# FederatedAI/FATE-LLM

Measured on AMD Instinct MI355X. Metric: GB/s param buffer reconstructed from (seed,scalar) list, device-resident, higher is better.
Workload: dtype bf16

## Files before the change

### fate-llm_amd/csrc/fks_device.hip

```cpp
#include <hip/hip_runtime.h>
#include <hip/hip_bf16.h>

#include <type_traits>

#include "fks_internal.h"
#include "fks_bitslice.h"
#define FKS_HD __device__ __forceinline__
#include "fks_libm.h"

constexpr int kDbMinWaves = 4;
constexpr int kZrUnroll = 2;
constexpr int kSm2MinWaves = 8;
constexpr int kBsFence = 8;
#ifndef FKS_BS_LAG
#define FKS_BS_LAG 36
#endif
#ifndef FKS_BS_R_VMEM
#define FKS_BS_R_VMEM 3
#endif
#ifndef FKS_BS_D16
#define FKS_BS_D16 1
#endif
#ifndef FKS_BS_G32
#define FKS_BS_G32 1
#endif
#ifndef FKS_BS_ROWMIN
#define FKS_BS_ROWMIN 1
#endif
#ifndef FKS_BS_FLIPMUX
#define FKS_BS_FLIPMUX 1
#endif
#ifndef FKS_PHX_VEC_ITEMS
#define FKS_PHX_VEC_ITEMS 8
#endif
#ifndef FKS_BS_WGTIME
#define FKS_BS_WGTIME 0
#endif

#include "fks_dev_lds.h"
#include "fks_dev_update.h"
#include "fks_dev_mt.h"
#include "fks_dev_zgen.h"
#include "fks_dev_irr.h"
#include "fks_dev_host.h"
#include "fks_kern_jump.h"
#include "fks_kern_apply.h"
#include "fks_kern_slice.h"
#include "fks_kern_irregular.h"
#include "fks_kern_philox.h"
#include "fks_kern_selfcheck.h"

namespace fks {

int launch_delta_apply(const DeltaApplyDesc* d, int n, int64_t max_numel, const float* delta, void* stream) {
  const int64_t blocks = std::min<int64_t>(std::max<int64_t>(1, (max_numel + 255) / 256), 2048);
  hipLaunchKernelGGL(fks_delta_apply_kernel, dim3((unsigned)blocks, (unsigned)n), dim3(256), 0, (hipStream_t)stream,
                     d, delta);
  return (int)hipGetLastError();
}

static size_t apply_lds_bytes() { return (size_t)kLdsTabBytes + (size_t)kLdsStBytes; }

int device_cu_count() {
  int dev = 0, n = 0;
  if (hipGetDevice(&dev) != hipSuccess) return 256;
  if (hipDeviceGetAttribute(&n, hipDeviceAttributeMultiprocessorCount, dev) != hipSuccess || n <= 0) return 256;
  return n;
}

template <int... Vs>
struct IntList {};
template <int... Vs, class F>
static int dispatch(IntList<Vs...>, int v, F&& f) {
  int r = -FKS_ENOTSUP;
  (void)((v == Vs && (r = f(std::integral_constant<int, Vs>{}), true)) || ...);
  return r;
}

int launch_jump(const JumpArgs& a, int nseeds, void* stream) {
  const size_t lds = sizeof(uint32_t) * (size_t)kJumpLds2Words;
  static PerDevice attr;
  if (int e = ensure_lds_attr(attr, &fks_jump_kernel, (int)lds)) return e;
  dim3 grid((unsigned)nseeds, (unsigned)((a.nchunks + a.chunks_per_wg - 1) / a.chunks_per_wg));
// ... 27 lines not shown
static int launch_apply_t(const ApplyArgs& a, void* stream) {
  if (a.nseeds == kMaxSeedsPerPass) return launch_apply_f<DT, MODE, true>(a, stream);
  if constexpr (DT == FKS_BF16) {
    if (a.zmode == 1 && a.nseeds == 1 && MODE == kModePerturb) return launch_small2<DT, MODE, 1>(a, stream);
    if (a.zmode == 2 && a.nseeds == 1 &&
        (MODE == kModePerturb || MODE == kModePerturbUpdate || MODE == kModeUpdate || MODE == kModeUpdateWd ||
         MODE == kModeUpdateNoWd || MODE == kModeUpdateWd0)) {
      hipLaunchKernelGGL((fks_zreplay_kernel<MODE>), dim3((unsigned)a.nchunks), dim3(kZrThreads), (size_t)3 * 1024,
                         (hipStream_t)stream, a);
      return (int)hipGetLastError();
    }
  }
  if (a.zmode == 2) return -FKS_ENOTSUP;
  if (a.nseeds <= kSmallK && DT != FKS_F16) return launch_small2<DT == FKS_F16 ? FKS_F32 : DT, MODE>(a, stream);
  if (a.nseeds <= kSmallK) return launch_apply_f<DT, MODE, false, true>(a, stream);
  return launch_apply_f<DT, MODE, false>(a, stream);
}

int launch_apply(int dtype, const ApplyArgs& a, void* stream) {
  if (a.nseeds < 1 || a.nseeds > kMaxSeedsPerPass || a.nchunks < 1) return -FKS_EINVAL;
  if (dtype == FKS_BF16) {
    int e = ensure_tables();
    if (e) return e;
  }
  using Modes = IntList<kModeUpdate, kModeUpdateWd, kModeUpdateNoWd, kModeUpdateWd0, kModePerturb, kModePerturbUpdate,
                        kModeWriteZ, kModeDelta>;
  return dispatch(IntList<FKS_F32, kDtF32Libm, FKS_BF16>{}, dtype, [&](auto dt) {
    return dispatch(Modes{}, a.mode,
                    [&](auto m) { return launch_apply_t<decltype(dt)::value, decltype(m)::value>(a, stream); });
  });
}

template <int MODE, bool FULL>
static int launch_apply_bs_m(const ApplyBsArgs& a, void* stream) {
  static PerDevice attr;
  if (int e = ensure_lds_attr(attr, &fks_apply_bs_kernel<MODE, FULL>, kBsLdsBytes)) return e;
  hipLaunchKernelGGL((fks_apply_bs_kernel<MODE, FULL>), dim3((unsigned)(a.split ? a.nchunks / 2 : a.nchunks)),
                     dim3(kBsThreads), kBsLdsBytes, (hipStream_t)stream, a);
  return (int)hipGetLastError();
}

template <int MODE>
static int launch_apply_bs_t(const ApplyBsArgs& a, void* stream) {
  const bool full = a.nseeds == (a.split ? kBsSeeds : kBsPassSeeds);
  return full ? launch_apply_bs_m<MODE, true>(a, stream) : launch_apply_bs_m<MODE, false>(a, stream);
}

int launch_apply_bs(const ApplyBsArgs& a, void* stream) {
  if (a.nseeds < 1 || a.nseeds > (a.split ? kBsSeeds : kBsPassSeeds) || a.nchunks < 1 ||
      (a.split && a.nchunks % 2))
    return -FKS_EINVAL;
  int e = ensure_tables();
  if (e) return e;
  return dispatch(IntList<kModeUpdate, kModeUpdateWd, kModeUpdateNoWd, kModeUpdateWd0, kModeDelta>{}, a.mode,
                  [&](auto m) { return launch_apply_bs_t<decltype(m)::value>(a, stream); });
}

template <int MODE>
static int launch_irregular_m(const IrrArgs& a, void* stream) {
  const size_t lds = (size_t)kIrrLogfOff + kLdsLogfBytes;
  static PerDevice attr;
  if (int e = ensure_lds_attr(attr, &fks_irregular_kernel<MODE>, (int)lds)) return e;
  hipLaunchKernelGGL((fks_irregular_kernel<MODE>), dim3((unsigned)a.nchunks), dim3(kApplyThreads), lds,
                     (hipStream_t)stream, a);
  return (int)hipGetLastError();
}

int launch_philox_fast_radius_check(uint32_t* counts, void* stream) {
  hipLaunchKernelGGL(fks_philox_fast_radius_kernel, dim3(kSqrtDomainBlocks), dim3(256), 0, (hipStream_t)stream, counts);
  return (int)hipGetLastError();
}

int launch_philox_radius_check(uint32_t* counts, void* stream) {
  hipLaunchKernelGGL(fks_philox_radius_kernel, dim3(kSqrtDomainBlocks), dim3(256), 0, (hipStream_t)stream, counts);
  return (int)hipGetLastError();
}

int launch_sqrt_domain_check(uint32_t* counts, void* stream) {
  hipLaunchKernelGGL(fks_sqrt_domain_kernel, dim3(kSqrtDomainBlocks), dim3(256), 0, (hipStream_t)stream, counts);
  return (int)hipGetLastError();
}

int device_max_threads_per_cu() {
  int dev = 0, n = 0;
  if (hipGetDevice(&dev) != hipSuccess) return 2048;
  if (hipDeviceGetAttribute(&n, hipDeviceAttributeMaxThreadsPerMultiProcessor, dev) != hipSuccess || n <= 0) return 2048;
  return n;
}

static int phx_vec_maxk() {
  static const int v = [] {
    const char* s = std::getenv("FKS_PHX_VEC_MAXK");
    return (s && *s) ? std::atoi(s) : kPhxSeeds;
  }();
  return v;
}

template <int MODE>
static int launch_philox_m(const PhiloxArgs& a, void* stream) {
  const int64_t items = a.item_hi - a.item_lo;
  if (items <= 0) return 0;
  if (a.nseeds <= phx_vec_maxk() && a.item_lo % kPhxVec == 0 && items % kPhxVec == 0) {
    const int64_t vitems = items / kPhxVec;
    const int64_t blocks = std::min<int64_t>((vitems + 255) / 256, (int64_t)device_cu_count() * 16);
    const size_t lds = a.nt <= kPhxLdsTensors ? sizeof(PhxTensor) * (size_t)a.nt : 0;
    hipLaunchKernelGGL((fks_philox_vec_kernel<MODE>), dim3((unsigned)blocks), dim3(256), lds, (hipStream_t)stream, a);
    return (int)hipGetLastError();
// ... 23 lines not shown
```

### fate-llm_amd/csrc/fks_host.h

```cpp
#pragma once

#include <algorithm>
#include <cstring>
#include <mutex>
#include <unordered_map>
#include <utility>

#include "fks_internal.h"
#include "fks_project_mt.h"
#include "fks_expand.h"

namespace fks {

inline size_t elem_size(int dtype) { return dtype == FKS_F32 ? 4 : 2; }
inline size_t align_up(size_t x, size_t a) { return (x + a - 1) / a * a; }
inline bool rocm_stream(const fks_tensor* t, int nt) { return nt > 0 && (t[0].flags & FKS_STREAM_ROCM) != 0; }
inline bool libm_flavour(const fks_tensor* t, int nt) { return nt > 0 && (t[0].flags & FKS_LIBM) != 0; }

void validate_basics(const fks_tensor* t, int nt);
void validate(const fks_tensor* t, int nt);
void check_shard(int shard, int nshards);

struct Layout {
  int64_t stream_len = 0;
  std::vector<DevSeg> segs[3];
  std::vector<DevRun> runs;
  std::vector<DevTiny> tiny;
  std::vector<int> seg_tensor[3], run_tensor, tiny_tensor;
  bool delta = false;
  bool end_cached = false;
  int64_t end_pair = 0;
};
inline size_t stor_size(const Layout& L, int dtype) { return L.delta ? 4 : elem_size(dtype); }
Layout make_layout(const fks_tensor* t, int nt, const double* scales = nullptr, uint64_t delta_base = 0);

struct BlockRange { int64_t lo, hi; };
BlockRange shard_blocks(int64_t stream_len, int shard, int nshards);
void clip_segments(Layout& L, BlockRange r);
inline int64_t block_of(int64_t w) { return w / kMtN; }

int plan_nchunks(int64_t nblocks, bool small, int cus);
int bs_nchunks(int64_t nblocks, int cus);
std::vector<int64_t> chunk_table(BlockRange r, int nchunks);

struct IrrChunks { std::vector<int64_t> lo, hi; };
std::vector<std::pair<int64_t, int64_t>> irregular_owner_intervals(const Layout& L);
IrrChunks irregular_chunks(const Layout& L, int cus);

struct HdrSizes {
  int reg_chunks = 0, irr_chunks = 0, nsegs = 0, nruns = 0, ntiny = 0;
  int bs_chunks = 0;
};
struct HdrLayout {
  size_t off_polys = 0, off_cb = 0, off_ipolys = 0, off_ilo = 0, off_ihi = 0, off_segs = 0, off_runs = 0,
         off_tiny = 0, off_bs_polys = 0, off_bs_cb = 0;
  size_t total = 0;
};

struct PlanInfo {
  HdrLayout H;
  HdrSizes Z;
  size_t seg_off[3] = {0, 0, 0};
  int nsegs[3] = {0, 0, 0};
  int wd_mode[3] = {kModeUpdate, kModeUpdate, kModeUpdate};
  bool have_reg = false, have_irr = false;
  bool have_bs = false;
  uint64_t chunk_hash = 0;
  int64_t reg_lo = 0, reg_hi = 0;
  uint64_t bf16_hash = 0;
  uint64_t bs_hash = 0;
};
struct PlanImage { std::vector<uint8_t> bytes; PlanInfo info; };
PlanImage plan_image(const fks_tensor* t, int nt, const double* scales, uint64_t delta_base, int shard, int nshards,
                     bool small, int cus);

constexpr size_t kWsStatesOff = 4096;
size_t ws_bytes_for(int chunks, int seeds_per_pass);
size_t workspace_total(const fks_tensor* t, int nt, int k, uint64_t delta_base, int cus);
struct ProjMtWs {
  size_t partial_off = 0, total = 0;
  int rows = 0;
  bool work = false;
  int entries = 0;
};
ProjMtWs project_mt_ws(const fks_tensor* t, int nt, int k, int shard, int nshards, int cus);
struct ProjMtMultiWs {
  ProjMtWs one;
  size_t inner_off = 0;
  size_t total = 0;
  int pass_vec = 0;
};
ProjMtMultiWs project_mt_multi_ws(const fks_tensor* t, int nt, int k, int nvec, int shard, int nshards, int cus);

template <class D>
int wd_form(const std::vector<D>& v, bool allow_wd0 = true) {
  size_t nwd = 0, nwd0 = 0;
  for (const D& x : v) {
    nwd += (x.flags & FKS_HAS_WD) ? 1 : 0;
    nwd0 += ((x.flags & FKS_HAS_WD) && x.wd == 0.0f) ? 1 : 0;
  }
  if (v.empty()) return kModeUpdate;
  if (nwd0 == v.size() && allow_wd0) return kModeUpdateWd0;
  return nwd == v.size() ? kModeUpdateWd : (nwd == 0 ? kModeUpdateNoWd : kModeUpdate);
}

float round_to_dtype(double v, int dtype);
inline float g_value(int value_kind, double v, int dtype) {
  return value_kind == FKS_VALUE_TENSOR ? round_to_dtype(v, dtype) : (float)v;
}

template <class T>
void key_put(std::vector<uint8_t>& k, const T& v) {
  const uint8_t* p = reinterpret_cast<const uint8_t*>(&v);
  k.insert(k.end(), p, p + sizeof(T));
}
uint64_t fnv1a(const std::vector<uint8_t>& b);

void mt_census(const fks_tensor* t, int nt, int shard, int nshards, int64_t* word_range, int64_t* written);
void cpu_generator_end(const fks_tensor* t, int nt, uint64_t seed, uint32_t* state624, int32_t* left, uint32_t* next,
// ... 118 lines not shown
```

### fate-llm_amd/csrc/fks_kern_slice.h

```cpp
#pragma once
#include <hip/hip_runtime.h>

#include "fks_internal.h"
#include "fks_bitslice.h"
#include "fks_dev_lds.h"
#include "fks_dev_update.h"
#include "fks_dev_zgen.h"

namespace fks {
namespace {

constexpr int kBsChunkBytes = kMtN * 16;
constexpr int kBsStateBytes = 8 * kBsChunkBytes;
constexpr int kBsTabBytes = 256 * 4 + 256 * 8;
constexpr uint32_t kBsFlagOff = kBsTabBytes + 2 * kBsStateBytes;
constexpr uint32_t kBsProgOff = kBsFlagOff + 8;
constexpr uint32_t kBsProg1Off = kBsProgOff + 4 * 6;
constexpr int kBsLdsBytes = (int)kBsProg1Off + 4 * 6;
static_assert(kBsLdsBytes <= 163840, "slice kernel LDS");
constexpr int kBsWaves = kBsHalfThreads / 64;
constexpr int kBsTaskWords = 128;

__device__ __forceinline__ void bs_store_row(uint32_t ra, const uint32_t (&x)[32]) {
#pragma unroll
// ... 29 lines not shown
                                  hipMemcpyDeviceToHost);
}
#endif

template <int MODE, bool FULL>
__global__ __launch_bounds__(kBsThreads, 1) void fks_apply_bs_kernel(ApplyBsArgs a) {
  extern __shared__ __attribute__((aligned(16))) uint32_t lds32[];
  if ((uint32_t)(size_t)(lds_u32_t*)lds32 != 0u) __builtin_trap();
  const int tid = threadIdx.x;
  const int lane = tid & 63;
#if FKS_BS_WGTIME
  if (tid == 0) g_bs_wgtime[blockIdx.x][0] = __builtin_amdgcn_s_memrealtime();
  auto stamp = [&]() { if (lane == 0) g_bs_wgtime[blockIdx.x][1 + (tid >> 6)] = __builtin_amdgcn_s_memrealtime(); };
#else
  auto stamp = [&]() {};
#endif
  const int half = __builtin_amdgcn_readfirstlane(tid >= kBsHalfThreads ? 1 : 0);
  const int ht = tid - half * kBsHalfThreads;
  const int hw = __builtin_amdgcn_readfirstlane(ht >> 6);
  const bool split = a.split != 0;
  const int c = split ? 2 * (int)blockIdx.x + half : (int)blockIdx.x;
  const int nA = FULL ? kBsSeeds : split ? a.nseeds : (a.nseeds + 1) / 2;
  const int nseeds = FULL ? kBsSeeds : (half && !split ? a.nseeds - nA : nA);
  const int sfirst = half && !split ? nA : 0;
  const int64_t b0 = a.chunk_block[split ? c : 2 * c], b1 = a.chunk_block[split ? c + 1 : 2 * c + 2];
  const int nwords = (int)(kMtN * (b1 - b0));
  const int ntask = (nwords + kBsTaskWords - 1) / kBsTaskWords;
  const uint32_t sbase = kBsTabBytes + (uint32_t)half * kBsStateBytes;
  const uint32_t flag = kBsFlagOff + 4u * (uint32_t)half;

  for (int i = tid; i < 256; i += kBsThreads) {
    reinterpret_cast<float*>((uint8_t*)lds32)[i] = c_tab_bf16[i];
    reinterpret_cast<float2*>((uint8_t*)lds32 + 1024)[i] = make_float2(c_tab_bf16[256 + i], c_tab_bf16[512 + i]);
  }
  for (int i = ht; i < kMtN; i += kBsHalfThreads) {
    uint32_t w[32];
#pragma unroll
    for (int k = 0; k < 32; k++)
      w[k] = k < nseeds ? a.states[((size_t)(a.use_slot ? a.slot[sfirst + k] : (uint32_t)(sfirst + k)) * a.nchunks + c) *
                                       kMtN + i]
                        : 0u;
    bs::transpose32(w);
    bs_store_row(sbase + 16u * (uint32_t)i, w);
  }
  if (ht == 0) lds32[flag / 4] = 0u;
  if (ht < kBsWaves) lds32[(half ? kBsProg1Off : kBsProgOff) / 4 + ht] = 0u;
  __syncthreads();
  if (nseeds == 0) return;

  const int toff = 16 * (lane >> 3) + (lane & 7);
  const bool flip = ((lane >> 3) & 1) != 0;
  const bool odd = (lane & 1) != 0;

  constexpr bool kWd0 = MODE == kModeUpdateWd0;
  constexpr bool kD16 = kWd0 && FKS_BS_D16 != 0;
  constexpr bool kG32 = kWd0 && FKS_BS_G32 != 0;
  constexpr bool kRowMin = kWd0 && FKS_BS_ROWMIN != 0;
  constexpr bool kFlipMux = kWd0 && FKS_BS_FLIPMUX != 0;
  uint32_t flipm = flip ? ~0u : 0u;
  if (kFlipMux) asm volatile("" : "+v"(flipm));

  float gk[kBsSeeds];
#pragma unroll
  for (int k = 0; k < kBsSeeds; k++) gk[k] = a.g[half ? k + sfirst : k];
  uint64_t gg[kBsSeeds / 2];
#pragma unroll
  for (int k = 0; k < kBsSeeds / 2; k++)
    gg[k] = (uint64_t)rfl(__float_as_uint(gk[2 * k])) | ((uint64_t)rfl(__float_as_uint(gk[2 * k + 1])) << 32);

  const int64_t wbase = (int64_t)kMtN * b0;
  int cur;
  {
    const int64_t s1 = wbase + (int64_t)kBsTaskWords * hw + toff;
    int lo = 0, hi = a.nsegs;
    while (lo < hi) {
      const int mid = (lo + hi) >> 1;
      if (a.segs[mid].start + a.segs[mid].numel <= s1) lo = mid + 1; else hi = mid;
    }
    cur = lo;
  }
  int64_t seg_start = INT64_MAX, seg_end = INT64_MAX;
  uint64_t seg_ptr = 0;
  float seg_lr = 0.0f, seg_wd = 0.0f;
  bool seg_wdf = false;
  constexpr int kEs = MODE == kModeDelta ? 4 : 2;
  constexpr bool kInc = MODE == kModeUpdateWd0;
  int seg_lo = INT32_MAX, seg_hi = INT32_MAX;
  uint64_t seg_org = 0;
  auto load_seg = [&]() {
    if (cur < a.nsegs) {
      const DevSeg sg = a.segs[cur];
      seg_start = sg.start;
      seg_end = sg.start + sg.numel;
      seg_ptr = sg.ptr;
      seg_lr = sg.lr;
      seg_wd = sg.wd;
      seg_wdf = (sg.flags & FKS_HAS_WD) != 0;
    } else {
      seg_start = seg_end = INT64_MAX;
    }
    if (kInc) {
      const int64_t lo = seg_start - wbase, hi = seg_end - wbase;
      seg_lo = (int)(lo < INT32_MIN ? INT32_MIN : lo > INT32_MAX ? INT32_MAX : lo);
      seg_hi = (int)(hi < INT32_MIN ? INT32_MIN : hi > INT32_MAX ? INT32_MAX : hi);
      seg_org = seg_ptr - (uint64_t)lo * kEs;
    }
    __builtin_amdgcn_s_waitcnt(0x0F70);
  };
  load_seg();

  using ST = Traits<MODE == kModeDelta ? FKS_F32 : FKS_BF16>;
  typedef typename ST::Pair Pair;
  struct Slot { uint64_t addr; float lr, wd; uint32_t wdf; Pair raw; uint32_t hi0, hi1; };
  auto fetch = [&](int n) -> Slot {
    Slot sl;
    const int u1 = kBsTaskWords * n + toff;
    if (kInc) {
      while (u1 >= seg_hi) { cur++; load_seg(); }
      const bool on = u1 < nwords && u1 >= seg_lo;
      sl.lr = seg_lr; sl.wd = seg_wd; sl.wdf = seg_wdf;
      sl.addr = on ? seg_org + (uint64_t)(uint32_t)(u1 + (odd && !kD16 ? 7 : 0)) * kEs : (uint64_t)(uintptr_t)a.sink;
      if (kD16) {
        sl.hi0 = Traits<FKS_BF16>::load_hi(sl.addr);
        sl.hi1 = Traits<FKS_BF16>::load_hi(sl.addr + 16);
        return sl;
      }
    } else {
      const int64_t s1 = wbase + u1;
      while (s1 >= seg_end) { cur++; load_seg(); }
      const bool on = u1 < nwords && s1 >= seg_start;
      sl.lr = seg_lr; sl.wd = seg_wd; sl.wdf = seg_wdf;
      sl.addr = on ? seg_ptr + (uint64_t)(s1 - seg_start + (odd ? 7 : 0)) * kEs : (uint64_t)(uintptr_t)a.sink;
    }
    sl.raw = ST::load_pair(sl.addr);
    return sl;
  };

  constexpr int kRowStep = kBsWaves * kBsTaskWords % kMtN;
  int row = (kBsTaskWords * hw + toff) % kMtN;
  auto wrap = [](uint32_t x) -> uint32_t {
    const uint32_t y = x - (uint32_t)kMtN;
    return x < y ? x : y;
  };
  uint32_t rofa = flip ? 8u : 0u, rofb = flip ? 0u : 8u;
  if (kRowMin) asm volatile("" : "+v"(rofa), "+v"(rofb));
  auto next_row = [&]() {
    if (!kInc) return;
    if (kRowMin) {
      row = (int)wrap((uint32_t)row + kRowStep);
      return;
    }
    row += kRowStep;
    if (row >= kMtN) row -= kMtN;
  };
  auto twist = [&](const int n, uint32_t (&oa)[8], uint32_t (&ob)[8]) {
    const int u1 = kBsTaskWords * n + toff;
    const bool valid = u1 < nwords;
    const int i1 = kRowMin ? row : valid ? (kInc ? row : u1 % kMtN) : 0;
    const int ia = kRowMin ? i1 + (int)rofa : flip ? i1 + 8 : i1, ib = kRowMin ? i1 + (int)rofb : flip ? i1 : i1 + 8;
    auto rows = [&](int i, uint32_t& av, uint32_t& am, uint32_t& au) {
      const int iv = kRowMin ? (int)wrap((uint32_t)i + 1u) : i + 1 < kMtN ? i + 1 : 0;
      const int im = kRowMin ? (int)wrap((uint32_t)i + kMtM) : i < kMtN - kMtM ? i + kMtM : i - (kMtN - kMtM);
      av = sbase + 16u * (uint32_t)iv;
      am = sbase + 16u * (uint32_t)im;
      au = sbase + 7u * kBsChunkBytes + 16u * (uint32_t)i + 12u;
    };
    uint32_t av1, am1, au1, av2, am2, au2;
    rows(ia, av1, am1, au1);
    rows(ib, av2, am2, au2);
    uint32_t M1[32], M2[32];
    const uint32_t U1 = lds_u32((int)au1), U2 = lds_u32((int)au2);
    u32x4_t va = lds_u4(av1), vb = lds_u4(av2), ma = lds_u4(am1), mb = lds_u4(am2);
    const uint32_t v0a = va.x, v0b = vb.x;
#pragma unroll
    for (int q = 0; q < 8; q++) {
      u32x4_t va2 = va, vb2 = vb, ma2 = ma, mb2 = mb;
      if (q < 7) {
        va2 = lds_u4(av1 + (q + 1) * kBsChunkBytes);
        vb2 = lds_u4(av2 + (q + 1) * kBsChunkBytes);
        ma2 = lds_u4(am1 + (q + 1) * kBsChunkBytes);
        mb2 = lds_u4(am2 + (q + 1) * kBsChunkBytes);
      }
      const uint32_t Va[5] = {va.x, va.y, va.z, va.w, va2.x};
      const uint32_t Vb[5] = {vb.x, vb.y, vb.z, vb.w, vb2.x};
      const uint32_t Ma[4] = {ma.x, ma.y, ma.z, ma.w}, Mb[4] = {mb.x, mb.y, mb.z, mb.w};
#pragma unroll
      for (int t = 0; t < 4; t++) {
        const int b = 4 * q + t;
        const bool am = ((bs::kMatrixA >> b) & 1u) != 0;
        uint32_t xa, xb;
        if (b < 30) { xa = Va[t + 1]; xb = Vb[t + 1]; }
        else if (b == 30) { xa = U1; xb = U2; }
        else { xa = 0u; xb = 0u; }
        M1[b] = am ? bs::xor3(Ma[t], xa, v0a) : (Ma[t] ^ xa);
        M2[b] = am ? bs::xor3(Mb[t], xb, v0b) : (Mb[t] ^ xb);
      }
      if (valid) {
        lds_st4(sbase + 16u * (uint32_t)ia + q * kBsChunkBytes, u32x4_t{M1[4 * q], M1[4 * q + 1], M1[4 * q + 2], M1[4 * q + 3]});
        lds_st4(sbase + 16u * (uint32_t)ib + q * kBsChunkBytes, u32x4_t{M2[4 * q], M2[4 * q + 1], M2[4 * q + 2], M2[4 * q + 3]});
      }
      va = va2; vb = vb2; ma = ma2; mb = mb2;
    }
    uint32_t o1[8], o2[8];
    bs::temper_low8(M1, o1);
    bs::temper_low8(M2, o2);
#pragma unroll
    for (int j = 0; j < 8; j++) {
      oa[j] = kFlipMux ? bs::mux(flipm, o2[j], o1[j]) : flip ? o2[j] : o1[j];
      ob[j] = kFlipMux ? bs::mux(flipm, o1[j], o2[j]) : flip ? o1[j] : o2[j];
    }
  };

  constexpr int kRv = kInc ? FKS_BS_R_VMEM : 0;
  static_assert(kRv >= 0 && kRv <= 8, "FKS_BS_R_VMEM");
  auto rv_slot = [](const int k) __attribute__((always_inline)) -> int {
    return (k & 7) < kRv ? (k >> 3) * kRv + (k & 7) : -1;
  };
  auto chain_head = [&](uint32_t (&oa)[8], uint32_t (&ob)[8], float (&rv)[4 * kRv + 1]) {
    bs::transpose8(oa);
    bs::transpose8(ob);
#pragma unroll
    for (int k = 0; k < kBsSeeds; k++)
      if (rv_slot(k) >= 0)
        rv[rv_slot(k)] =
            *reinterpret_cast<const float*>(reinterpret_cast<const char*>(c_tab_bf16) + bs_index<2>(oa[k & 7], k >> 3));
  };
  auto chain = [&](const Slot& sl, uint32_t (&oa)[8], uint32_t (&ob)[8], const float (&rv)[4 * kRv + 1]) {
    if (kRv == 0) {
      bs::transpose8(oa);
      bs::transpose8(ob);
    }
    f32x2_t p;
    if (kD16) {
      p.x = __uint_as_float(sl.hi0);
      p.y = __uint_as_float(sl.hi1);
    } else {
      const uint32_t keep = odd ? ST::hi(sl.raw) : ST::lo(sl.raw);
      const uint32_t got = swap_adjacent(odd ? ST::lo(sl.raw) : ST::hi(sl.raw));
      p.x = ST::cvt(odd ? got : keep);
      p.y = ST::cvt(odd ? keep : got);
    }
    auto z_of = [&](const int k) __attribute__((always_inline)) -> f32x2_t {
      const float r = rv_slot(k) >= 0 ? rv[rv_slot(k)] : lds_f32(bs_index<2>(oa[k & 7], k >> 3));
      const f32x2_t rr = {r, r}, zero = {0.0f, 0.0f};
      const f32x2_t cs = lds_f32x2(1024u + bs_index<3>(ob[k & 7], k >> 3));
      return rnd2<FKS_BF16>(__builtin_elementwise_fma(rr, cs, zero));
    };
    {
#pragma unroll
      for (int k = 0; k < kBsSeeds; k++) {
        if (FULL || k < nseeds) {
          if (kG32)
            p = apply_tail<FKS_BF16, MODE>(p, rnd2<FKS_BF16>(k & 1 ? pk_mul_half<1>(gg[k >> 1], z_of(k)) : pk_mul_half<0>(gg[k >> 1], z_of(k))),
                                           sl.lr, sl.wd, sl.wdf != 0);
          else
            p = apply_pair<FKS_BF16, MODE>(p, z_of(k), gk[k], sl.lr, sl.wd, sl.wdf != 0, 0.0f);
        }
        if ((k % kBsFence) == kBsFence - 1) asm volatile("" ::: "memory");
      }
    }
    if (kD16) {
      Traits<FKS_BF16>::store_hi(sl.addr, __float_as_uint(p.x));
      Traits<FKS_BF16>::store_hi(sl.addr + 16, __float_as_uint(p.y));
      return;
    }
    const uint32_t b1v = ST::bits(p.x), b2v = ST::bits(p.y);
    const uint32_t back = swap_adjacent(odd ? b1v : b2v);
    const Pair out = odd ? ST::pack(back, b2v) : ST::pack(b1v, back);
    ST::store_pair(sl.addr, out);
  };

  const bool ordered = !split;
  const uint32_t prog = kBsProgOff + 4u * (uint32_t)hw;
  auto publish_stored = [&](const int m) {
    asm volatile("" ::: "memory");
    __builtin_amdgcn_s_waitcnt(0x0F70);
    if (lane == 0) *(volatile lds_u32_t*)(size_t)prog = (uint32_t)m + 1u;
  };
  auto await_stored = [&](const int m) {
    if (m >= ntask) return;
    const uint32_t pm = kBsProgOff + 4u * (uint32_t)(m % kBsWaves);
    while (__builtin_amdgcn_readfirstlane(bs_flag_load(pm)) < (uint32_t)m + 1u) __builtin_amdgcn_s_sleep(1);
    asm volatile("" ::: "memory");
  };
  static_assert(FKS_BS_LAG == 0 || FKS_BS_LAG > 2 * kBsWaves, "FKS_BS_LAG: half 1 trails by 12 tasks");
  constexpr bool kLag = FKS_BS_LAG > 0 && (MODE == kModeUpdateWd || MODE == kModeUpdate);
  const uint32_t prog1 = kBsProg1Off + 4u * (uint32_t)hw;
  auto publish_applied = [&](const int m) {
    if (lane == 0) *(volatile lds_u32_t*)(size_t)prog1 = (uint32_t)m + 1u;
  };
  auto await_applied = [&](const int m) {
    if (m < 0) return;
    const uint32_t pm = kBsProg1Off + 4u * (uint32_t)(m % kBsWaves);
    while (__builtin_amdgcn_readfirstlane(bs_flag_load(pm)) < (uint32_t)m + 1u) __builtin_amdgcn_s_sleep(1);
  };

  auto task = [&](const int n, const Slot& sl, Slot& nx) {
    uint32_t oa[8], ob[8];
    if (kLag && ordered && half == 0) await_applied(n - FKS_BS_LAG);
    __builtin_amdgcn_s_setprio(2);
    while (__builtin_amdgcn_readfirstlane(bs_flag_load(flag)) < (uint32_t)n) __builtin_amdgcn_s_sleep(0);
    asm volatile("" ::: "memory");
    twist(n, oa, ob);
    if (lane == 0) bs_flag_store(flag, (uint32_t)n + 1u);
    __builtin_amdgcn_s_setprio(0);
    if (ordered && half == 0) {
      if (n >= kBsWaves) publish_stored(n - kBsWaves);
    } else if (ordered) {
      await_stored(n + kBsWaves);
    }
    float rv[4 * kRv + 1];
    if (kRv > 0) chain_head(oa, ob, rv);
    nx = fetch(n + kBsWaves);
    chain(sl, oa, ob, rv);
    if (kLag && ordered && half) publish_applied(n);
  };

  if (hw >= ntask) { stamp(); return; }
  if (ordered && half) await_stored(hw);
  Slot s0 = fetch(hw), s1;
  int n = hw;
  for (;;) {
    task(n, s0, s1);
    if (n + kBsWaves >= ntask) break;
    n += kBsWaves;
    next_row();
    task(n, s1, s0);
    if (n + kBsWaves >= ntask) break;
    n += kBsWaves;
    next_row();
  }
  if (ordered && half == 0) publish_stored(n);
  stamp();
}

}
}
```

### fate-llm_amd/csrc/fks_layout.cpp

```cpp
#include <cmath>

#include "fks_host.h"

namespace fks {

static void check_list(const fks_tensor* t, int nt) {
  if (nt < 0 || (nt > 0 && !t)) throw Error(-FKS_EINVAL, "bad tensor list");
}
static void check_basics(const fks_tensor& x, int i) {
  if (x.numel < 0) throw Error(-FKS_EINVAL, "tensor " + std::to_string(i) + ": negative numel");
  if (x.dtype != FKS_F32 && x.dtype != FKS_BF16 && x.dtype != FKS_F16)
    throw Error(-FKS_EINVAL, "tensor " + std::to_string(i) + ": unsupported dtype code " + std::to_string(x.dtype));
  if (x.numel > 0 && (!x.data || ((uintptr_t)x.data % elem_size(x.dtype)) != 0))
    throw Error(-FKS_EINVAL, "tensor " + std::to_string(i) + ": null or misaligned data pointer");
}

void validate_basics(const fks_tensor* t, int nt) {
  check_list(t, nt);
  for (int i = 0; i < nt; i++) check_basics(t[i], i);
}

void validate(const fks_tensor* t, int nt) {
  check_list(t, nt);
  for (int i = 0; i < nt; i++) {
// ... 248 lines not shown
  return w;
}

uint64_t fnv1a(const std::vector<uint8_t>& b) {
  uint64_t h = 1469598103934665603ull;
  for (uint8_t c : b) h = (h ^ c) * 1099511628211ull;
  return h;
}

constexpr bool kWd0F32Mode = false;

PlanImage plan_image(const fks_tensor* t, int nt, const double* scales, uint64_t delta_base, int shard, int nshards,
                     bool small, int cus) {
  Layout L = make_layout(t, nt, scales, delta_base);
  const BlockRange br = shard_blocks(L.stream_len, shard, nshards);
  clip_segments(L, br);
  PlanImage img;
  PlanInfo& C = img.info;
  C.have_reg = nsegs_total(L) > 0;
  C.have_irr = !L.runs.empty() || !L.tiny.empty();
  std::vector<int64_t> cb, bcb;
  if (C.have_reg) cb = chunk_table(br, plan_nchunks(std::max<int64_t>(1, br.hi - br.lo), small, cus));
  C.have_bs = !small && !L.segs[FKS_BF16].empty();
  if (C.have_bs) {
    bcb = chunk_table(br, bs_nchunks(br.hi - br.lo, cus));
    const int n = (int)bcb.size() - 1;
    for (int c = 0; C.have_bs && c < n; c++)
      if ((bcb[(size_t)std::min(c + 2, n)] - bcb[(size_t)c]) * kMtN >= ((int64_t)1 << 31)) C.have_bs = false;
    if (!C.have_bs) bcb.clear();
  }
  const IrrChunks IC = irregular_chunks(L, cus);
  std::vector<uint64_t> polys, ipolys, bpolys;
  if (!cb.empty()) jump_polys_for_blocks(std::vector<int64_t>(cb.begin(), cb.end() - 1), polys);
  if (C.have_irr) jump_polys_for_blocks(IC.lo, ipolys);
  if (!bcb.empty()) jump_polys_for_blocks(std::vector<int64_t>(bcb.begin(), bcb.end() - 1), bpolys);
  C.Z.reg_chunks = cb.empty() ? 0 : (int)cb.size() - 1;
  C.Z.irr_chunks = (int)IC.lo.size();
  C.Z.nsegs = nsegs_total(L);
  C.Z.nruns = (int)L.runs.size();
  C.Z.ntiny = (int)L.tiny.size();
  C.Z.bs_chunks = bcb.empty() ? 0 : (int)bcb.size() - 1;
  auto put = [&](size_t& off, const auto& v) {
    off = img.bytes.size();
    const size_t bytes = sizeof(v[0]) * v.size();
    img.bytes.resize(align_up(off + std::max<size_t>(bytes, 1), 256), 0);
    if (bytes) std::memcpy(img.bytes.data() + off, v.data(), bytes);
  };
  std::vector<DevSeg> segs;
  for (int d = 0; d < 3; d++) {
    C.nsegs[d] = (int)L.segs[d].size();
    C.wd_mode[d] = wd_form(L.segs[d], d != FKS_F32 || kWd0F32Mode);
    segs.insert(segs.end(), L.segs[d].begin(), L.segs[d].end());
  }
  put(C.H.off_polys, polys);
  put(C.H.off_cb, cb);
  put(C.H.off_ipolys, ipolys);
  put(C.H.off_ilo, IC.lo);
  put(C.H.off_ihi, IC.hi);
  put(C.H.off_segs, segs);
  put(C.H.off_runs, L.runs);
  put(C.H.off_tiny, L.tiny);
  put(C.H.off_bs_polys, bpolys);
  put(C.H.off_bs_cb, bcb);
  C.H.total = img.bytes.size();
  C.seg_off[0] = C.H.off_segs;
  for (int d = 1; d < 3; d++) C.seg_off[d] = C.seg_off[d - 1] + sizeof(DevSeg) * L.segs[d - 1].size();
  std::vector<uint8_t> ck;
  for (int64_t b : cb) key_put(ck, b);
  key_put(ck, (int64_t)-1);
  for (int64_t b : IC.lo) key_put(ck, b);
  C.chunk_hash = fnv1a(ck);
  std::vector<uint8_t> bk;
  for (const DevSeg& sg : L.segs[FKS_BF16]) {
    key_put(bk, sg.start);
    key_put(bk, sg.numel);
  }
  C.bf16_hash = fnv1a(bk);
  std::vector<uint8_t> sk;
  for (int64_t b : bcb) key_put(sk, b);
  C.bs_hash = bcb.empty() ? 0 : (fnv1a(sk) | 1u);
  if (C.have_reg && !cb.empty()) {
    C.reg_lo = cb.front();
    C.reg_hi = cb.back();
  }
  return img;
}

void mt_census(const fks_tensor* t, int nt, int shard, int nshards, int64_t* word_range, int64_t* written) {
  Layout L = make_layout(t, nt);
  const BlockRange br = shard_blocks(L.stream_len, shard, nshards);
  clip_segments(L, br);
  if (word_range) {
    word_range[0] = br.lo * kMtN;
    word_range[1] = br.hi * kMtN;
  }
  if (!written) return;
  for (int i = 0; i < nt; i++) written[i] = 0;
  for (int d = 0; d < 3; d++)
    for (size_t j = 0; j < L.segs[d].size(); j++) written[L.seg_tensor[d][j]] += L.segs[d][j].numel;
  for (size_t j = 0; j < L.runs.size(); j++)
    written[L.run_tensor[j]] += std::max<int64_t>(0, std::min(L.runs[j].limit, L.runs[j].numel));
  for (size_t j = 0; j < L.tiny.size(); j++) written[L.tiny_tensor[j]] += 1;
}

void cpu_generator_end(const fks_tensor* t, int nt, uint64_t seed, uint32_t* state624, int32_t* left, uint32_t* next,
                       int32_t* normal_valid, double* normal) {
// ... 99 lines not shown
```

### fate-llm_amd/csrc/fks_run.cpp

```cpp
#include <hip/hip_runtime.h>

#include <cmath>
#include <cstdlib>

#include "fks_host.h"

namespace fks {
namespace {

struct Prof {
  bool on = false;
  std::vector<std::pair<hipEvent_t, hipEvent_t>> ev[2];
};
Prof g_prof;
std::mutex g_prof_mu;

template <class F>
int timed(int which, void* stream, F&& launch) {
  std::unique_lock<std::mutex> lk(g_prof_mu);
  if (!g_prof.on) {
    lk.unlock();
    return launch();
  }
  hipEvent_t a, b;
// ... 109 lines not shown
  const bool use_bs = C->have_bs && k >= kBsMinSeeds && (mode == kModeUpdate || mode == kModeDelta);
  size_t need = ws_bytes_for(std::max(C->Z.reg_chunks, C->Z.irr_chunks), std::min(per_pass, k));
  if (use_bs) need = std::max(need, ws_bytes_for(C->Z.bs_chunks, std::min(kBsSeeds, k)));
  if (!workspace || ws_bytes < need)
    throw Error(-FKS_EINVAL, "workspace too small: need " + std::to_string(need) + " bytes, got " +
                                 std::to_string(ws_bytes));
  uint8_t* ws = static_cast<uint8_t*>(workspace);
  const uint8_t* hdr = static_cast<const uint8_t*>(C->dev);
  uint32_t* states = reinterpret_cast<uint32_t*>(ws + kWsStatesOff);
  ZCache* Zc = nullptr;
  int zmode = 0;
  const bool z_mode_ok = mode == kModePerturb || mode == kModePerturbUpdate || mode == kModeUpdate;
  if (k == 1 && small && !use_bs && C->have_reg && C->nsegs[FKS_BF16] > 0 && z_mode_ok) {
    Zc = z_cache(stream, (size_t)kSm2ZidxBytesPerBlock * (size_t)(C->reg_hi - C->reg_lo));
    if (Zc) {
      if (Zc->valid && Zc->seed == seeds[0] && Zc->bf16_hash == C->bf16_hash && Zc->lo <= C->reg_lo &&
          C->reg_hi <= Zc->hi) {
        zmode = 2;
      } else if (mode == kModePerturb) {
        zmode = 1;
        Zc->valid = false;
        Zc->lo = C->reg_lo;
        Zc->hi = C->reg_hi;
        Zc->bf16_hash = C->bf16_hash;
      } else {
        Zc = nullptr;
      }
    }
  }
  uint32_t* reg_states = states;
  uint32_t* irr_states = states;
  bool reg_cached = false, irr_cached = false, reg_jumped = false;
  WinCache* W = nullptr;
  if (k == 1 && !use_bs) {
    const size_t reg_words = (size_t)kMtN * (C->have_reg ? C->Z.reg_chunks : 0);
    const size_t irr_words = (size_t)kMtN * (C->have_irr ? C->Z.irr_chunks : 0);
    W = win_cache(stream, sizeof(uint32_t) * std::max<size_t>(reg_words + irr_words, 1));
    if (W) {
      reg_states = static_cast<uint32_t*>(W->b.buf);
      irr_states = reg_states + reg_words;
      const bool hit = W->valid && W->seed == seeds[0] && W->chunk_hash == C->chunk_hash;
      reg_cached = irr_cached = hit;
      W->valid = false;
    }
  }
  RecordAfter z_after{Zc ? &Zc->b : nullptr, stream}, w_after{W ? &W->b : nullptr, stream};
  auto gval = [&](int s, int d) { return g_value(value_kind, values[s], d); };
  if (use_bs) {
    int slices = 2;
    if (const char* e = std::getenv("FKS_BS_SLICES")) slices = (e[0] == '1') ? 1 : 2;
    const int per_pass = slices == 2 ? kBsPassSeeds : kBsSeeds;
    JWin* J = (slices == 2 && k > kBsSeeds) ? jw_cache(stream, C->bs_hash, C->Z.bs_chunks / kBsChunksPerWg) : nullptr;
    RecordAfter j_after{J ? &J->b : nullptr, stream, J};
    for (int s0 = 0; s0 < k; s0 += per_pass) {
      const int nb = std::min(per_pass, k - s0);
      const bool split = nb <= kBsSeeds;
      const int nch = split ? C->Z.bs_chunks : C->Z.bs_chunks / kBsChunksPerWg;
      JumpArgs ja = jump_args(seeds + s0, nb, hdr, C->H.off_bs_polys, C->H.off_bs_cb, states, nch);
      ApplyBsArgs ba{};
      int njump = nb;
      ba.states = states;
      if (J && !split) {
        jw_assign(J->sets, seeds + s0, nb, ba.slot, ja.seeds, ja.slot, njump);
        ja.states = static_cast<uint32_t*>(J->b.buf);
        ba.states = ja.states;
        ja.use_slot = ba.use_slot = 1;
      }
      ja.stride = split ? 1 : kBsChunksPerWg;
      ja.chunks_per_wg = std::max(1, std::min(njump * nch >= 4096 ? 32 : 16, nch));
      if (njump > 0) check_launch(timed(1, stream, [&] { return launch_jump(ja, njump, stream); }), "fks_jump_kernel");
      for (int j = 0; j < nb; j++) ba.g[j] = gval(s0 + j, FKS_BF16);
      ba.segs = reinterpret_cast<const DevSeg*>(hdr + C->seg_off[FKS_BF16]);
      ba.chunk_block = ja.chunk_block;
      ba.sink = reinterpret_cast<uint64_t*>(ws);
      ba.nsegs = C->nsegs[FKS_BF16];
      ba.nchunks = nch;
      ba.split = split ? 1 : 0;
      ba.nseeds = nb;
      ba.mode = mode == kModeUpdate ? C->wd_mode[FKS_BF16] : mode;
      check_launch(timed(0, stream, [&] { return launch_apply_bs(ba, stream); }), "fks_apply_bs_kernel");
    }
    (void)j_after.record();
  }
  bool reg_rest = false;
  for (int d = 0; d < 3; d++) reg_rest = reg_rest || (C->nsegs[d] && !(use_bs && d == FKS_BF16));
  for (int s0 = 0; s0 < k; s0 += kMaxSeedsPerPass) {
    const int nb = std::min(kMaxSeedsPerPass, k - s0);
    if (reg_rest) {
      JumpArgs ja = jump_args(seeds + s0, nb, hdr, C->H.off_polys, C->H.off_cb, reg_states, C->Z.reg_chunks);
      ja.chunks_per_wg = jump_chunks_per_wg(nb, C->Z.reg_chunks, dc.cus);
      const bool need_windows = zmode != 2 || C->nsegs[FKS_F32] > 0 || C->nsegs[FKS_F16] > 0;
      if (!reg_cached && need_windows) {
        check_launch(timed(1, stream, [&] { return launch_jump(ja, nb, stream); }), "fks_jump_kernel");
        reg_jumped = true;
      }
      for (int d = 0; d < 3; d++) {
        if (!C->nsegs[d] || (use_bs && d == FKS_BF16)) continue;
        ApplyArgs aa{};
        aa.states = reg_states;
        for (int j = 0; j < nb; j++) aa.g[j] = gval(s0 + j, d);
        aa.segs = reinterpret_cast<const DevSeg*>(hdr + C->seg_off[d]);
        aa.chunk_block = ja.chunk_block;
        aa.sink = reinterpret_cast<uint64_t*>(ws);
        aa.gdev = gdev;
        if (Zc && d == FKS_BF16) {
          aa.zidx = static_cast<uint32_t*>(Zc->b.buf);
          aa.zlo = Zc->lo;
          aa.zmode = zmode;
        }
        aa.nsegs = C->nsegs[d];
        aa.nchunks = C->Z.reg_chunks;
        aa.nseeds = nb;
        aa.mode = mode == kModeUpdate ? C->wd_mode[d] : mode;
        const int dd = (d == FKS_F32 && libm) ? kDtF32Libm : d;
        check_launch(timed(0, stream, [&] { return launch_apply(dd, aa, stream); }), "fks_apply_kernel");
      }
    }
    if (C->have_irr) {
      JumpArgs ja = jump_args(seeds + s0, nb, hdr, C->H.off_ipolys, C->H.off_ilo, irr_states, C->Z.irr_chunks);
      ja.chunks_per_wg = std::max(1, std::min(32, C->Z.irr_chunks));
      if (!irr_cached) check_launch(timed(1, stream, [&] { return launch_jump(ja, nb, stream); }), "fks_jump_kernel");
      IrrArgs ia{};
      ia.states = irr_states;
      for (int d = 0; d < 3; d++)
        for (int j = 0; j < nb; j++) ia.g[d][j] = gval(s0 + j, d);
      ia.runs = reinterpret_cast<const DevRun*>(hdr + C->H.off_runs);
      ia.tiny = reinterpret_cast<const DevTiny*>(hdr + C->H.off_tiny);
      ia.chunk_lo = ja.chunk_block;
      ia.chunk_hi = reinterpret_cast<const int64_t*>(hdr + C->H.off_ihi);
      ia.gdev = gdev;
      ia.nruns = C->Z.nruns;
      ia.ntiny = C->Z.ntiny;
// ... 489 lines not shown
```

Before: 1.291.

## Add positive-zero weight-decay mode with lookahead table loads in bitslice apply kernel

Adds a kModeUpdateWdPos0 specialization, selected on the host when all bf16 segments have a +0 weight decay and gradient and lr bounds rule out overflow. In that mode the kernel canonicalizes the parameter once with an fma so the per-seed update can skip the decay arithmetic. It also software-pipelines the r/cs LDS table loads with a lookahead window and precomputes twist LDS addresses before the flag wait. The aim is to hide LDS latency and trim VALU work in the inner seed loop, at the cost of more registers and an extra template instantiation.

```diff
diff --git a/fate-llm_amd/csrc/fks_device.hip b/fate-llm_amd/csrc/fks_device.hip
--- a/fate-llm_amd/csrc/fks_device.hip
+++ b/fate-llm_amd/csrc/fks_device.hip
@@ -29,6 +29,12 @@
 #endif
 #ifndef FKS_BS_FLIPMUX
 #define FKS_BS_FLIPMUX 1
+#endif
+#ifndef FKS_BS_LOOK
+#define FKS_BS_LOOK 16
+#endif
+#ifndef FKS_BS_H1
+#define FKS_BS_H1 1
 #endif
 #ifndef FKS_PHX_VEC_ITEMS
 #define FKS_PHX_VEC_ITEMS 8
@@ -162,7 +168,7 @@
     return -FKS_EINVAL;
   int e = ensure_tables();
   if (e) return e;
-  return dispatch(IntList<kModeUpdate, kModeUpdateWd, kModeUpdateNoWd, kModeUpdateWd0, kModeDelta>{}, a.mode,
+  return dispatch(IntList<kModeUpdate, kModeUpdateWd, kModeUpdateNoWd, kModeUpdateWd0, kModeUpdateWdPos0, kModeDelta>{}, a.mode,
                   [&](auto m) { return launch_apply_bs_t<decltype(m)::value>(a, stream); });
 }
 
diff --git a/fate-llm_amd/csrc/fks_host.h b/fate-llm_amd/csrc/fks_host.h
--- a/fate-llm_amd/csrc/fks_host.h
+++ b/fate-llm_amd/csrc/fks_host.h
@@ -65,6 +65,8 @@
   int wd_mode[3] = {kModeUpdate, kModeUpdate, kModeUpdate};
   bool have_reg = false, have_irr = false;
   bool have_bs = false;
+  bool bs_wd_pos0 = false;
+  float bs_max_lr = 0.0f;
   uint64_t chunk_hash = 0;
   int64_t reg_lo = 0, reg_hi = 0;
   uint64_t bf16_hash = 0;
diff --git a/fate-llm_amd/csrc/fks_kern_slice.h b/fate-llm_amd/csrc/fks_kern_slice.h
--- a/fate-llm_amd/csrc/fks_kern_slice.h
+++ b/fate-llm_amd/csrc/fks_kern_slice.h
@@ -105,7 +105,8 @@
   const bool flip = ((lane >> 3) & 1) != 0;
   const bool odd = (lane & 1) != 0;
 
-  constexpr bool kWd0 = MODE == kModeUpdateWd0;
+  constexpr bool kPos0 = MODE == kModeUpdateWdPos0;
+  constexpr bool kWd0 = MODE == kModeUpdateWd0 || kPos0;
   constexpr bool kD16 = kWd0 && FKS_BS_D16 != 0;
   constexpr bool kG32 = kWd0 && FKS_BS_G32 != 0;
   constexpr bool kRowMin = kWd0 && FKS_BS_ROWMIN != 0;
@@ -137,7 +138,7 @@
   float seg_lr = 0.0f, seg_wd = 0.0f;
   bool seg_wdf = false;
   constexpr int kEs = MODE == kModeDelta ? 4 : 2;
-  constexpr bool kInc = MODE == kModeUpdateWd0;
+  constexpr bool kInc = kWd0;
   int seg_lo = INT32_MAX, seg_hi = INT32_MAX;
   uint64_t seg_org = 0;
   auto load_seg = [&]() {
@@ -206,6 +207,22 @@
     row += kRowStep;
     if (row >= kMtN) row -= kMtN;
   };
+  struct TwAddr { uint32_t av1, am1, au1, av2, am2, au2, sa, sb; };
+  constexpr bool kH1 = kPos0 && kRowMin && FKS_BS_H1 != 0;
+  TwAddr pre{};
+  auto tw_pre = [&]() {
+    const uint32_t ia = (uint32_t)row + rofa, ib = (uint32_t)row + rofb;
+    pre.av1 = sbase + 16u * wrap(ia + 1u);
+    pre.am1 = sbase + 16u * wrap(ia + kMtM);
+    pre.au1 = sbase + 7u * kBsChunkBytes + 16u * ia + 12u;
+    pre.av2 = sbase + 16u * wrap(ib + 1u);
+    pre.am2 = sbase + 16u * wrap(ib + kMtM);
+    pre.au2 = sbase + 7u * kBsChunkBytes + 16u * ib + 12u;
+    pre.sa = sbase + 16u * ia;
+    pre.sb = sbase + 16u * ib;
+    asm volatile("" : "+v"(pre.av1), "+v"(pre.am1), "+v"(pre.au1), "+v"(pre.av2), "+v"(pre.am2), "+v"(pre.au2),
+                 "+v"(pre.sa), "+v"(pre.sb));
+  };
   auto twist = [&](const int n, uint32_t (&oa)[8], uint32_t (&ob)[8]) {
     const int u1 = kBsTaskWords * n + toff;
     const bool valid = u1 < nwords;
@@ -221,6 +238,10 @@
     uint32_t av1, am1, au1, av2, am2, au2;
     rows(ia, av1, am1, au1);
     rows(ib, av2, am2, au2);
+    if (kH1) {
+      av1 = pre.av1; am1 = pre.am1; au1 = pre.au1;
+      av2 = pre.av2; am2 = pre.am2; au2 = pre.au2;
+    }
     uint32_t M1[32], M2[32];
     const uint32_t U1 = lds_u32((int)au1), U2 = lds_u32((int)au2);
     u32x4_t va = lds_u4(av1), vb = lds_u4(av2), ma = lds_u4(am1), mb = lds_u4(am2);
@@ -249,8 +270,8 @@
         M2[b] = am ? bs::xor3(Mb[t], xb, v0b) : (Mb[t] ^ xb);
       }
       if (valid) {
-        lds_st4(sbase + 16u * (uint32_t)ia + q * kBsChunkBytes, u32x4_t{M1[4 * q], M1[4 * q + 1], M1[4 * q + 2], M1[4 * q + 3]});
-        lds_st4(sbase + 16u * (uint32_t)ib + q * kBsChunkBytes, u32x4_t{M2[4 * q], M2[4 * q + 1], M2[4 * q + 2], M2[4 * q + 3]});
+        lds_st4((kH1 ? pre.sa : sbase + 16u * (uint32_t)ia) + q * kBsChunkBytes, u32x4_t{M1[4 * q], M1[4 * q + 1], M1[4 * q + 2], M1[4 * q + 3]});
+        lds_st4((kH1 ? pre.sb : sbase + 16u * (uint32_t)ib) + q * kBsChunkBytes, u32x4_t{M2[4 * q], M2[4 * q + 1], M2[4 * q + 2], M2[4 * q + 3]});
       }
       va = va2; vb = vb2; ma = ma2; mb = mb2;
     }
@@ -293,25 +314,57 @@
       p.x = ST::cvt(odd ? got : keep);
       p.y = ST::cvt(odd ? keep : got);
     }
+    if (kPos0) {
+      const f32x2_t zero = {0.0f, 0.0f};
+      p = __builtin_elementwise_fma(zero, p, p);
+    }
     auto z_of = [&](const int k) __attribute__((always_inline)) -> f32x2_t {
       const float r = rv_slot(k) >= 0 ? rv[rv_slot(k)] : lds_f32(bs_index<2>(oa[k & 7], k >> 3));
       const f32x2_t rr = {r, r}, zero = {0.0f, 0.0f};
       const f32x2_t cs = lds_f32x2(1024u + bs_index<3>(ob[k & 7], k >> 3));
       return rnd2<FKS_BF16>(__builtin_elementwise_fma(rr, cs, zero));
     };
+#if FKS_BS_LOOK > 0
+    constexpr int kLook = kPos0 ? FKS_BS_LOOK : 0;
+    static_assert(kLook <= kBsSeeds, "FKS_BS_LOOK");
+    float wr[kLook + 1];
+    f32x2_t wcs[kLook + 1];
+    auto look = [&](const int k, const int s) __attribute__((always_inline)) {
+      wr[s] = rv_slot(k) >= 0 ? rv[rv_slot(k)] : lds_f32(bs_index<2>(oa[k & 7], k >> 3));
+      wcs[s] = lds_f32x2(1024u + bs_index<3>(ob[k & 7], k >> 3));
+    };
+#pragma unroll
+    for (int k = 0; k < kLook; k++) {
+      wr[k] = 0.0f;
+      wcs[k] = f32x2_t{0.0f, 0.0f};
+      if (FULL || k < nseeds) look(k, k);
+    }
+    auto z_la = [&](const int k) __attribute__((always_inline)) -> f32x2_t {
+      const int s = k % (kLook > 0 ? kLook : 1);
+      const f32x2_t rr = {wr[s], wr[s]}, zero = {0.0f, 0.0f}, cs = wcs[s];
+      if (k + kLook < kBsSeeds && (FULL || k + kLook < nseeds)) {
+        look(k + kLook, s);
+      }
+      return rnd2<FKS_BF16>(__builtin_elementwise_fma(rr, cs, zero));
+    };
+#define FKS_BS_Z(k) (kLook > 0 ? z_la(k) : z_of(k))
+#else
+#define FKS_BS_Z(k) z_of(k)
+#endif
     {
 #pragma unroll
       for (int k = 0; k < kBsSeeds; k++) {
         if (FULL || k < nseeds) {
           if (kG32)
-            p = apply_tail<FKS_BF16, MODE>(p, rnd2<FKS_BF16>(k & 1 ? pk_mul_half<1>(gg[k >> 1], z_of(k)) : pk_mul_half<0>(gg[k >> 1], z_of(k))),
+            p = apply_tail<FKS_BF16, MODE>(p, rnd2<FKS_BF16>(k & 1 ? pk_mul_half<1>(gg[k >> 1], FKS_BS_Z(k)) : pk_mul_half<0>(gg[k >> 1], FKS_BS_Z(k))),
                                            sl.lr, sl.wd, sl.wdf != 0);
           else
-            p = apply_pair<FKS_BF16, MODE>(p, z_of(k), gk[k], sl.lr, sl.wd, sl.wdf != 0, 0.0f);
+            p = apply_pair<FKS_BF16, MODE>(p, FKS_BS_Z(k), gk[k], sl.lr, sl.wd, sl.wdf != 0, 0.0f);
         }
         if ((k % kBsFence) == kBsFence - 1) asm volatile("" ::: "memory");
       }
     }
+#undef FKS_BS_Z
     if (kD16) {
       Traits<FKS_BF16>::store_hi(sl.addr, __float_as_uint(p.x));
       Traits<FKS_BF16>::store_hi(sl.addr + 16, __float_as_uint(p.y));
@@ -351,6 +404,7 @@
   auto task = [&](const int n, const Slot& sl, Slot& nx) {
     uint32_t oa[8], ob[8];
     if (kLag && ordered && half == 0) await_applied(n - FKS_BS_LAG);
+    if (kH1) tw_pre();
     __builtin_amdgcn_s_setprio(2);
     while (__builtin_amdgcn_readfirstlane(bs_flag_load(flag)) < (uint32_t)n) __builtin_amdgcn_s_sleep(0);
     asm volatile("" ::: "memory");
diff --git a/fate-llm_amd/csrc/fks_layout.cpp b/fate-llm_amd/csrc/fks_layout.cpp
--- a/fate-llm_amd/csrc/fks_layout.cpp
+++ b/fate-llm_amd/csrc/fks_layout.cpp
@@ -324,6 +324,13 @@
     C.wd_mode[d] = wd_form(L.segs[d], d != FKS_F32 || kWd0F32Mode);
     segs.insert(segs.end(), L.segs[d].begin(), L.segs[d].end());
   }
+  C.bs_wd_pos0 = C.wd_mode[FKS_BF16] == kModeUpdateWd0;
+  for (const DevSeg& sg : L.segs[FKS_BF16]) {
+    uint32_t wb;
+    std::memcpy(&wb, &sg.wd, 4);
+    C.bs_wd_pos0 = C.bs_wd_pos0 && wb == 0u && std::isfinite(sg.lr);
+    C.bs_max_lr = std::max(C.bs_max_lr, std::fabs(sg.lr));
+  }
   put(C.H.off_polys, polys);
   put(C.H.off_cb, cb);
   put(C.H.off_ipolys, ipolys);
diff --git a/fate-llm_amd/csrc/fks_run.cpp b/fate-llm_amd/csrc/fks_run.cpp
--- a/fate-llm_amd/csrc/fks_run.cpp
+++ b/fate-llm_amd/csrc/fks_run.cpp
@@ -185,6 +185,17 @@
     const int per_pass = slices == 2 ? kBsPassSeeds : kBsSeeds;
     JWin* J = (slices == 2 && k > kBsSeeds) ? jw_cache(stream, C->bs_hash, C->Z.bs_chunks / kBsChunksPerWg) : nullptr;
     RecordAfter j_after{J ? &J->b : nullptr, stream, J};
+    int bs_mode = mode == kModeUpdate ? C->wd_mode[FKS_BF16] : mode;
+    if (bs_mode == kModeUpdateWd0 && C->bs_wd_pos0 && !env_on("FKS_BS_KEEP_WD_FMA")) {
+      double gmax = 0.0;
+      bool finite = std::isfinite((double)C->bs_max_lr);
+      for (int j = 0; j < k && finite; j++) {
+        const float g = gval(j, FKS_BF16);
+        finite = finite && std::isfinite(g);
+        gmax = std::max(gmax, (double)std::fabs(g));
+      }
+      if (finite && gmax * 6.67 <= 1e37 && gmax * 6.67 * (double)C->bs_max_lr <= 1e30) bs_mode = kModeUpdateWdPos0;
+    }
     for (int s0 = 0; s0 < k; s0 += per_pass) {
       const int nb = std::min(per_pass, k - s0);
       const bool split = nb <= kBsSeeds;
@@ -210,7 +221,7 @@
       ba.nchunks = nch;
       ba.split = split ? 1 : 0;
       ba.nseeds = nb;
-      ba.mode = mode == kModeUpdate ? C->wd_mode[FKS_BF16] : mode;
+      ba.mode = bs_mode;
       check_launch(timed(0, stream, [&] { return launch_apply_bs(ba, stream); }), "fks_apply_bs_kernel");
     }
     (void)j_after.record();
```

Result: faster. 1.315 (median of 6 runs) (+1.8%).
